# salute-developers/GigaAM

Measured on NVIDIA H100. Metric: utterances/sec (10 s audio, v2_ctc), higher is better.
Workload: dtype f16 tensor-core operands, f32 accumulate/residual/norm/head

## Files before the change

### gigaam_b200/csrc/attention_sm90.cu

```cuda
#include "kernels.h"
#include "launch.cuh"
#include "ptx.cuh"

namespace gam {
namespace {

constexpr int kMaxKB = 6;
constexpr int kTileBytes = 128 * 128;
constexpr int kThreads = 256;
constexpr float kLazyLog2 = 8.0f;
constexpr int kBarBytes = 128;

__device__ __forceinline__ float ex2(float x) {
  float y;
  asm("ex2.approx.ftz.f32 %0, %1;" : "=f"(y) : "f"(x));
  return y;
}

struct AttnParams {
  int T, nkb;
  const int* klen;
  const int* cu;
  __half* out;
  int ld_out, dk;
  float scale_log2;
};

template <int KS>
__global__ void __launch_bounds__(kThreads) attention_kernel(const __grid_constant__ CUtensorMap tmap_qkv, const AttnParams p) {
  extern __shared__ uint8_t smem_raw[];
  uint8_t* smem = reinterpret_cast<uint8_t*>((reinterpret_cast<uintptr_t>(smem_raw) + 1023) & ~uintptr_t(1023));
  const int nst = min(p.nkb, kMaxKB);
  uint8_t* sQ = smem;
  uint8_t* sK = smem + kTileBytes;
  uint8_t* sV = sK + nst * kTileBytes;
  uint64_t* bars = reinterpret_cast<uint64_t*>(sV + nst * kTileBytes);
  uint64_t* q_full = bars;
  uint64_t* kv_full = bars + 1;

  const int qt = blockIdx.x, h = blockIdx.y, b = blockIdx.z;
  const int klen = p.klen != nullptr ? min(max(__ldg(p.klen + b), 0), p.T) : p.T;
  const int kb_valid = (klen + 127) >> 7;
  if (p.cu != nullptr && qt >= kb_valid) return;
  const int row0 = p.cu != nullptr ? __ldg(p.cu + b) : b * p.T;
  const int qlim = p.cu != nullptr ? klen : p.T;
  const int nk = max(1, kb_valid);
  const int dmodel = p.ld_out;

  auto issue_block = [&](int kb, int st) {
    ptx::mbar_arrive_expect_tx(&kv_full[st], 2 * kTileBytes);
    ptx::tma_load_2d(sK + st * kTileBytes, &tmap_qkv, &kv_full[st], dmodel + h * p.dk, row0 + kb * 128);
    ptx::tma_load_2d(sV + st * kTileBytes, &tmap_qkv, &kv_full[st], 2 * dmodel + h * p.dk, row0 + kb * 128);
  };
  if (threadIdx.x == 0) {
    const int npre = nk < kMaxKB ? nk : kMaxKB;
    ptx::prefetch_tmap(&tmap_qkv);
    ptx::mbar_init(q_full, 1);
#pragma unroll
    for (int i = 0; i < kMaxKB; ++i)
      if (i < npre) ptx::mbar_init(&kv_full[i], 1);
    ptx::fence_mbar_init();
    ptx::mbar_arrive_expect_tx(q_full, kTileBytes);
    ptx::tma_load_2d(sQ, &tmap_qkv, q_full, h * p.dk, row0 + qt * 128);
#pragma unroll
    for (int kb = 0; kb < kMaxKB; ++kb)
      if (kb < npre) issue_block(kb, kb);
  }
  __syncthreads();

  const int warp = threadIdx.x >> 5, lane = threadIdx.x & 31;
  const int g = lane >> 2, t4 = lane & 3;
  uint32_t qa[KS][4];
  ptx::mbar_wait(q_full, 0);
#pragma unroll
  for (int kk = 0; kk < KS; ++kk)
    ptx::ldsm_x4(ptx::smem_u32(sQ) + ptx::sw128_off(warp * 16 + (lane & 15), kk * 16 + (lane >> 4) * 8), qa[kk][0], qa[kk][1],
                 qa[kk][2], qa[kk][3]);

  float o[2 * KS][4];
#pragma unroll
  for (int i = 0; i < 2 * KS; ++i) o[i][0] = o[i][1] = o[i][2] = o[i][3] = 0.f;
  float mc[2] = {0.f, 0.f};
  float sum[2] = {0.f, 0.f};

  for (int kb = 0; kb < nk; ++kb) {
    const int nvalid = max(min(klen - kb * 128, 128), 0);
    const int st = kb % kMaxKB;
    ptx::mbar_wait(&kv_full[st], (kb / kMaxKB) & 1);
    uint8_t* kt = sK + st * kTileBytes;
    uint8_t* vt = sV + st * kTileBytes;
    if (nvalid < 128) {
      __syncthreads();
      for (int i = threadIdx.x; i < (128 - nvalid) * 8; i += kThreads)
        reinterpret_cast<uint4*>(vt + nvalid * 128)[i] = make_uint4(0u, 0u, 0u, 0u);
      __syncthreads();
    }
    const int nch = (nvalid + 15) >> 4;

    float s[16][4];
#pragma unroll
    for (int j = 0; j < 8; ++j) {
      s[2 * j][0] = s[2 * j][1] = s[2 * j][2] = s[2 * j][3] = 0.f;
      s[2 * j + 1][0] = s[2 * j + 1][1] = s[2 * j + 1][2] = s[2 * j + 1][3] = 0.f;
      if (j < nch) {
#pragma unroll
        for (int kk = 0; kk < KS; ++kk) {
          uint32_t b0, b1, b2, b3;
          ptx::ldsm_x4(ptx::smem_u32(kt) + ptx::sw128_off(16 * j + (lane & 7) + ((lane >> 4) << 3), kk * 16 + ((lane >> 3) & 1) * 8),
                       b0, b1, b2, b3);
          ptx::mma_16816(s[2 * j], qa[kk], b0, b1);
          ptx::mma_16816(s[2 * j + 1], qa[kk], b2, b3);
        }
      }
    }

    float bm[2] = {-INFINITY, -INFINITY};
#pragma unroll
    for (int i = 0; i < 16; ++i) {
#pragma unroll
      for (int e = 0; e < 4; ++e)
        if (8 * i + 2 * t4 + (e & 1) < nvalid) bm[e >> 1] = fmaxf(bm[e >> 1], s[i][e]);
    }
#pragma unroll
    for (int r = 0; r < 2; ++r) {
      bm[r] = fmaxf(bm[r], __shfl_xor_sync(0xffffffffu, bm[r], 1));
      bm[r] = fmaxf(bm[r], __shfl_xor_sync(0xffffffffu, bm[r], 2));
      const float bml = bm[r] * p.scale_log2;
      if (kb == 0) {
        mc[r] = bm[r] == -INFINITY ? 0.f : bml;
      } else if (bml > mc[r] + kLazyLog2) {
        const float corr = ex2(mc[r] - bml);
        mc[r] = bml;
        sum[r] *= corr;
#pragma unroll
        for (int i = 0; i < 2 * KS; ++i) {
          o[i][2 * r] *= corr;
          o[i][2 * r + 1] *= corr;
        }
      }
    }

#pragma unroll
    for (int j = 0; j < 8; ++j) {
      if (j < nch) {
        uint32_t pa[4];
#pragma unroll
        for (int u = 0; u < 2; ++u) {
#pragma unroll
          for (int r = 0; r < 2; ++r) {
            const int key = 16 * j + 8 * u + 2 * t4;
            const float p0 = key < nvalid ? ex2(fmaf(s[2 * j + u][2 * r], p.scale_log2, -mc[r])) : 0.f;
            const float p1 = key + 1 < nvalid ? ex2(fmaf(s[2 * j + u][2 * r + 1], p.scale_log2, -mc[r])) : 0.f;
            const __half2 hh = __floats2half2_rn(p0, p1);
            const float2 pr = __half22float2(hh);
            sum[r] += pr.x + pr.y;
            pa[2 * u + r] = *reinterpret_cast<const uint32_t*>(&hh);
          }
        }
#pragma unroll
        for (int dd = 0; dd < KS; ++dd) {
          uint32_t b0, b1, b2, b3;
          ptx::ldsm_x4_t(ptx::smem_u32(vt) + ptx::sw128_off(16 * j + (lane & 7) + (((lane >> 3) & 1) << 3), dd * 16 + ((lane >> 4) << 3)),
                         b0, b1, b2, b3);
          ptx::mma_16816(o[2 * dd], pa, b0, b1);
          ptx::mma_16816(o[2 * dd + 1], pa, b2, b3);
        }
      }
    }
    if (kb + kMaxKB < nk) {
      __syncthreads();
      if (threadIdx.x == 0) issue_block(kb + kMaxKB, st);
    }
  }

#pragma unroll
  for (int r = 0; r < 2; ++r) {
    sum[r] += __shfl_xor_sync(0xffffffffu, sum[r], 1);
    sum[r] += __shfl_xor_sync(0xffffffffu, sum[r], 2);
    const float inv = sum[r] > 0.f ? 1.0f / sum[r] : 0.f;
    const int q = qt * 128 + warp * 16 + g + 8 * r;
    if (q < qlim) {
      __half* dst = p.out + (static_cast<size_t>(row0) + q) * p.ld_out + h * p.dk + 2 * t4;
#pragma unroll
      for (int i = 0; i < 2 * KS; ++i) {
        const __half2 hh = __floats2half2_rn(o[i][2 * r] * inv, o[i][2 * r + 1] * inv);
        *reinterpret_cast<__half2*>(dst + 8 * i) = hh;
      }
    }
  }
}

template <int KS>
int launch_ks(const CUtensorMap* tmap_qkv, const AttnParams& p, int B, int H, cudaStream_t s) {
  const int smem = (1 + 2 * (p.nkb < kMaxKB ? p.nkb : kMaxKB)) * kTileBytes + kBarBytes + 1024;
  static PerDeviceOnce attr_once;
  if (attr_once.first() &&
      cudaFuncSetAttribute(attention_kernel<KS>, cudaFuncAttributeMaxDynamicSharedMemorySize, (1 + 2 * kMaxKB) * kTileBytes + kBarBytes + 1024) !=
          cudaSuccess)
    return -2;
  return launch_k(attention_kernel<KS>, dim3(p.nkb, H, B), dim3(kThreads), smem, s, *tmap_qkv, p) == cudaSuccess ? 0 : -2;
}

}

int launch_attention(const CUtensorMap* tmap_qkv, const int* klen, const int* cu, __half* out, int B, int T, int H, int dk,
                     int d_model, cudaStream_t s) {
  const int nkb = (T + 127) / 128;
  if (nkb <= 0 || dk % 16 != 0 || dk > 48 || (cu != nullptr && klen == nullptr)) return -1;
  AttnParams p;
  p.T = T;
  p.nkb = nkb;
  p.klen = klen;
  p.cu = cu;
  p.out = out;
  p.ld_out = d_model;
  p.dk = dk;
  p.scale_log2 = 1.4426950408889634f / sqrtf(static_cast<float>(dk));
  switch (dk / 16) {
    case 1: return launch_ks<1>(tmap_qkv, p, B, H, s);
    case 2: return launch_ks<2>(tmap_qkv, p, B, H, s);
    default: return launch_ks<3>(tmap_qkv, p, B, H, s);
  }
}

}
```

### gigaam_b200/csrc/ptx.cuh

```cuda
#pragma once
#include <cuda.h>
#include <cuda_fp16.h>
#include <cuda_runtime.h>
#include <stdint.h>

namespace gam {
namespace ptx {

__device__ __forceinline__ uint32_t smem_u32(const void* p) {
  return static_cast<uint32_t>(__cvta_generic_to_shared(p));
}

__device__ __forceinline__ uint32_t lane_id() {
  uint32_t l;
  asm volatile("mov.u32 %0, %%laneid;" : "=r"(l));
  return l;
}

__device__ __forceinline__ bool elect_one() {
  uint32_t pred = 0;
  asm volatile(
      "{\n\t"
      ".reg .pred P;\n\t"
      "elect.sync _|P, 0xffffffff;\n\t"
      "selp.u32 %0, 1, 0, P;\n\t"
      "}\n"
      : "=r"(pred));
  return pred != 0;
}

__device__ __forceinline__ void mbar_init(uint64_t* bar, uint32_t count) {
  asm volatile("mbarrier.init.shared::cta.b64 [%0], %1;" ::"r"(smem_u32(bar)), "r"(count));
}
__device__ __forceinline__ void fence_mbar_init() {
  asm volatile("fence.mbarrier_init.release.cluster;" ::: "memory");
}
__device__ __forceinline__ void fence_proxy_async_smem() {
  asm volatile("fence.proxy.async.shared::cta;" ::: "memory");
}
__device__ __forceinline__ void mbar_arrive(uint64_t* bar) {
  asm volatile("mbarrier.arrive.shared::cta.b64 _, [%0];" ::"r"(smem_u32(bar)) : "memory");
}
__device__ __forceinline__ void mbar_arrive_expect_tx(uint64_t* bar, uint32_t bytes) {
  asm volatile("mbarrier.arrive.expect_tx.shared::cta.b64 _, [%0], %1;" ::"r"(smem_u32(bar)),
               "r"(bytes)
               : "memory");
}
__device__ __forceinline__ bool mbar_try_wait(uint64_t* bar, uint32_t parity) {
  uint32_t ok;
  asm volatile(
      "{\n\t"
      ".reg .pred P;\n\t"
      "mbarrier.try_wait.parity.shared::cta.b64 P, [%1], %2;\n\t"
      "selp.u32 %0, 1, 0, P;\n\t"
      "}\n"
      : "=r"(ok)
      : "r"(smem_u32(bar)), "r"(parity)
      : "memory");
  return ok != 0;
}
__device__ __forceinline__ void mbar_wait(uint64_t* bar, uint32_t parity) {
  while (!mbar_try_wait(bar, parity)) {
  }
}

__device__ __forceinline__ void prefetch_tmap(const CUtensorMap* m) {
  asm volatile("prefetch.tensormap [%0];" ::"l"(reinterpret_cast<uint64_t>(m)) : "memory");
}
__device__ __forceinline__ void tma_load_2d(void* smem, const CUtensorMap* m, uint64_t* bar, int c0,
                                            int c1) {
  asm volatile(
      "cp.async.bulk.tensor.2d.shared::cluster.global.mbarrier::complete_tx::bytes [%0], [%1, {%3, "
      "%4}], [%2];" ::"r"(smem_u32(smem)),
      "l"(reinterpret_cast<uint64_t>(m)), "r"(smem_u32(bar)), "r"(c0), "r"(c1)
      : "memory");
}
__device__ __forceinline__ void tma_load_2d_multicast(void* smem, const CUtensorMap* m, uint64_t* bar, int c0, int c1,
                                                      uint16_t cta_mask) {
  asm volatile(
      "cp.async.bulk.tensor.2d.shared::cluster.global.mbarrier::complete_tx::bytes.multicast::cluster [%0], [%1, {%3, "
      "%4}], [%2], %5;" ::"r"(smem_u32(smem)),
      "l"(reinterpret_cast<uint64_t>(m)), "r"(smem_u32(bar)), "r"(c0), "r"(c1), "h"(cta_mask)
      : "memory");
}
__device__ __forceinline__ void tma_load_3d(void* smem, const CUtensorMap* m, uint64_t* bar, int c0, int c1, int c2) {
  asm volatile(
      "cp.async.bulk.tensor.3d.shared::cluster.global.mbarrier::complete_tx::bytes [%0], [%1, {%3, "
      "%4, %5}], [%2];" ::"r"(smem_u32(smem)),
      "l"(reinterpret_cast<uint64_t>(m)), "r"(smem_u32(bar)), "r"(c0), "r"(c1), "r"(c2)
      : "memory");
}

__device__ __forceinline__ void tma_load_4d(void* smem, const CUtensorMap* m, uint64_t* bar, int c0,
                                            int c1, int c2, int c3) {
  asm volatile(
      "cp.async.bulk.tensor.4d.shared::cluster.global.mbarrier::complete_tx::bytes [%0], [%1, {%3, "
      "%4, %5, %6}], [%2];" ::"r"(smem_u32(smem)),
      "l"(reinterpret_cast<uint64_t>(m)), "r"(smem_u32(bar)), "r"(c0), "r"(c1), "r"(c2), "r"(c3)
      : "memory");
}
__device__ __forceinline__ void tma_store_2d(const CUtensorMap* m, const void* smem, int c0, int c1) {
  asm volatile(
      "cp.async.bulk.tensor.2d.global.shared::cta.bulk_group [%0, {%2, %3}], [%1];" ::"l"(
          reinterpret_cast<uint64_t>(m)),
      "r"(smem_u32(smem)), "r"(c0), "r"(c1)
      : "memory");
}
__device__ __forceinline__ void tma_store_commit() {
  asm volatile("cp.async.bulk.commit_group;" ::: "memory");
}
template <int N>
__device__ __forceinline__ void tma_store_wait_read() {
  asm volatile("cp.async.bulk.wait_group.read %0;" ::"n"(N) : "memory");
}
template <int N>
__device__ __forceinline__ void tma_store_wait() {
  asm volatile("cp.async.bulk.wait_group %0;" ::"n"(N) : "memory");
}

template <int N>
__device__ __forceinline__ void named_bar_sync(int id) {
  asm volatile("bar.sync %0, %1;" ::"r"(id), "n"(N) : "memory");
}

template <int kRegs>
__device__ __forceinline__ void setmaxnreg_dec() {
  asm volatile("setmaxnreg.dec.sync.aligned.u32 %0;" ::"n"(kRegs));
}
template <int kRegs>
__device__ __forceinline__ void setmaxnreg_inc() {
  asm volatile("setmaxnreg.inc.sync.aligned.u32 %0;" ::"n"(kRegs));
}

__device__ __forceinline__ uint32_t mapa_u32(uint32_t smem_addr, uint32_t cta) {
  uint32_t r;
  asm volatile("mapa.shared::cluster.u32 %0, %1, %2;" : "=r"(r) : "r"(smem_addr), "r"(cta));
  return r;
}
__device__ __forceinline__ uint32_t cluster_ctarank() {
  uint32_t r;
  asm volatile("mov.u32 %0, %%cluster_ctarank;" : "=r"(r));
  return r;
}
__device__ __forceinline__ void cluster_sync() {
  asm volatile("barrier.cluster.arrive.release.aligned;\n\tbarrier.cluster.wait.acquire.aligned;" ::: "memory");
}
__device__ __forceinline__ void mbar_arrive_cluster(uint64_t* bar, uint32_t cta) {
  asm volatile("mbarrier.arrive.shared::cluster.b64 _, [%0];" ::"r"(mapa_u32(smem_u32(bar), cta)) : "memory");
}
__device__ __forceinline__ void st_async_v4(uint32_t remote_addr, uint32_t remote_bar, uint32_t a, uint32_t b, uint32_t c,
                                            uint32_t d) {
  asm volatile("st.async.weak.shared::cluster.mbarrier::complete_tx::bytes.v4.b32 [%0], {%1, %2, %3, %4}, [%5];" ::"r"(remote_addr),
               "r"(a), "r"(b), "r"(c), "r"(d), "r"(remote_bar)
               : "memory");
}
__device__ __forceinline__ uint64_t make_wgmma_desc_sw128(uint32_t smem_addr) {
  uint64_t d = 0;
  d |= static_cast<uint64_t>((smem_addr & 0x3FFFF) >> 4);
  d |= static_cast<uint64_t>(1) << 16;
  d |= static_cast<uint64_t>(1024 >> 4) << 32;
  d |= static_cast<uint64_t>(1) << 62;
  return d;
}
__device__ __forceinline__ void wgmma_fence() { asm volatile("wgmma.fence.sync.aligned;" ::: "memory"); }
__device__ __forceinline__ void wgmma_commit() { asm volatile("wgmma.commit_group.sync.aligned;" ::: "memory"); }
template <int N>
__device__ __forceinline__ void wgmma_wait() {
  asm volatile("wgmma.wait_group.sync.aligned %0;" ::"n"(N) : "memory");
}
__device__ __forceinline__ void wgmma_m64n256k16_f16(float* d, uint64_t desc_a, uint64_t desc_b, uint32_t scale_d) {
  asm volatile(
      "{\n\t"
      ".reg .pred p;\n\t"
      "setp.ne.b32 p, %130, 0;\n\t"
      "wgmma.mma_async.sync.aligned.m64n256k16.f32.f16.f16 "
      "{%0, %1, %2, %3, %4, %5, %6, %7, %8, %9, %10, %11, %12, %13, %14, %15, %16, %17, %18, %19, %20, %21, %22, %23, %24, %25, %26, %27, %28, %29, %30, %31, %32, %33, %34, %35, %36, %37, %38, %39, %40, %41, %42, %43, %44, %45, %46, %47, %48, %49, %50, %51, %52, %53, %54, %55, %56, %57, %58, %59, %60, %61, %62, %63, %64, %65, %66, %67, %68, %69, %70, %71, %72, %73, %74, %75, %76, %77, %78, %79, %80, %81, %82, %83, %84, %85, %86, %87, %88, %89, %90, %91, %92, %93, %94, %95, %96, %97, %98, %99, %100, %101, %102, %103, %104, %105, %106, %107, %108, %109, %110, %111, %112, %113, %114, %115, %116, %117, %118, %119, %120, %121, %122, %123, %124, %125, %126, %127}, "
      "%128, %129, p, 1, 1, 0, 0;\n\t"
      "}\n"
      : "+f"(d[0]), "+f"(d[1]), "+f"(d[2]), "+f"(d[3]), "+f"(d[4]), "+f"(d[5]), "+f"(d[6]), "+f"(d[7]), "+f"(d[8]), "+f"(d[9]), "+f"(d[10]), "+f"(d[11]), "+f"(d[12]), "+f"(d[13]), "+f"(d[14]), "+f"(d[15]), "+f"(d[16]), "+f"(d[17]), "+f"(d[18]), "+f"(d[19]), "+f"(d[20]), "+f"(d[21]), "+f"(d[22]), "+f"(d[23]), "+f"(d[24]), "+f"(d[25]), "+f"(d[26]), "+f"(d[27]), "+f"(d[28]), "+f"(d[29]), "+f"(d[30]), "+f"(d[31]), "+f"(d[32]), "+f"(d[33]), "+f"(d[34]), "+f"(d[35]), "+f"(d[36]), "+f"(d[37]), "+f"(d[38]), "+f"(d[39]), "+f"(d[40]), "+f"(d[41]), "+f"(d[42]), "+f"(d[43]), "+f"(d[44]), "+f"(d[45]), "+f"(d[46]), "+f"(d[47]), "+f"(d[48]), "+f"(d[49]), "+f"(d[50]), "+f"(d[51]), "+f"(d[52]), "+f"(d[53]), "+f"(d[54]), "+f"(d[55]), "+f"(d[56]), "+f"(d[57]), "+f"(d[58]), "+f"(d[59]), "+f"(d[60]), "+f"(d[61]), "+f"(d[62]), "+f"(d[63]), "+f"(d[64]), "+f"(d[65]), "+f"(d[66]), "+f"(d[67]), "+f"(d[68]), "+f"(d[69]), "+f"(d[70]), "+f"(d[71]), "+f"(d[72]), "+f"(d[73]), "+f"(d[74]), "+f"(d[75]), "+f"(d[76]), "+f"(d[77]), "+f"(d[78]), "+f"(d[79]), "+f"(d[80]), "+f"(d[81]), "+f"(d[82]), "+f"(d[83]), "+f"(d[84]), "+f"(d[85]), "+f"(d[86]), "+f"(d[87]), "+f"(d[88]), "+f"(d[89]), "+f"(d[90]), "+f"(d[91]), "+f"(d[92]), "+f"(d[93]), "+f"(d[94]), "+f"(d[95]), "+f"(d[96]), "+f"(d[97]), "+f"(d[98]), "+f"(d[99]), "+f"(d[100]), "+f"(d[101]), "+f"(d[102]), "+f"(d[103]), "+f"(d[104]), "+f"(d[105]), "+f"(d[106]), "+f"(d[107]), "+f"(d[108]), "+f"(d[109]), "+f"(d[110]), "+f"(d[111]), "+f"(d[112]), "+f"(d[113]), "+f"(d[114]), "+f"(d[115]), "+f"(d[116]), "+f"(d[117]), "+f"(d[118]), "+f"(d[119]), "+f"(d[120]), "+f"(d[121]), "+f"(d[122]), "+f"(d[123]), "+f"(d[124]), "+f"(d[125]), "+f"(d[126]), "+f"(d[127])
      : "l"(desc_a), "l"(desc_b), "r"(scale_d));
}

__device__ __forceinline__ void ldsm_x4(uint32_t addr, uint32_t& r0, uint32_t& r1, uint32_t& r2, uint32_t& r3) {
  asm volatile("ldmatrix.sync.aligned.m8n8.x4.shared.b16 {%0, %1, %2, %3}, [%4];"
               : "=r"(r0), "=r"(r1), "=r"(r2), "=r"(r3)
               : "r"(addr));
}
__device__ __forceinline__ void ldsm_x4_t(uint32_t addr, uint32_t& r0, uint32_t& r1, uint32_t& r2, uint32_t& r3) {
  asm volatile("ldmatrix.sync.aligned.m8n8.x4.trans.shared.b16 {%0, %1, %2, %3}, [%4];"
               : "=r"(r0), "=r"(r1), "=r"(r2), "=r"(r3)
               : "r"(addr));
}
__device__ __forceinline__ void mma_16816(float* d, const uint32_t* a, uint32_t b0, uint32_t b1) {
  asm volatile(
      "mma.sync.aligned.m16n8k16.row.col.f32.f16.f16.f32 {%0, %1, %2, %3}, {%4, %5, %6, %7}, {%8, %9}, "
      "{%0, %1, %2, %3};"
      : "+f"(d[0]), "+f"(d[1]), "+f"(d[2]), "+f"(d[3])
      : "r"(a[0]), "r"(a[1]), "r"(a[2]), "r"(a[3]), "r"(b0), "r"(b1));
}
__device__ __forceinline__ uint32_t sw128_off(int row, int col) {
  return static_cast<uint32_t>(row * 128 + ((((col >> 3) ^ row) & 7) << 4));
}
__device__ __forceinline__ uint32_t sw128_off_f32(int row, int col) {
  return static_cast<uint32_t>(row * 128 + ((((col >> 2) ^ row) & 7) << 4));
}

}
}
```

Measured before the change: 2774.

## Rewrite attention as persistent warp-specialized WGMMA kernel with TMA producer warp

The attention kernel now runs as a persistent grid sized to SM occupancy. One producer warpgroup streams double-buffered Q tiles and a 6-stage K/V ring via TMA, synchronised with full/empty mbarriers. Two consumer warpgroups compute QK^T and PV with wgmma (PV takes the A operand from registers), and the next block's QK^T is issued before the softmax of the current one so they overlap. This removes per-CTA launch overhead, block-wide syncthreads and ldmatrix+mma.sync issue costs, at the price of register pressure (240 regs per consumer thread), one CTA per SM, and more complex phase bookkeeping.

```diff
diff --git a/gigaam_b200/csrc/attention_sm90.cu b/gigaam_b200/csrc/attention_sm90.cu
--- a/gigaam_b200/csrc/attention_sm90.cu
+++ b/gigaam_b200/csrc/attention_sm90.cu
@@ -5,11 +5,12 @@
 namespace gam {
 namespace {
 
-constexpr int kMaxKB = 6;
+constexpr int kStages = 6;
 constexpr int kTileBytes = 128 * 128;
-constexpr int kThreads = 256;
+constexpr int kThreads = 384;
 constexpr float kLazyLog2 = 8.0f;
 constexpr int kBarBytes = 128;
+constexpr int kSmemBytes = (2 + 2 * kStages) * kTileBytes + kBarBytes + 1024;
 
 __device__ __forceinline__ float ex2(float x) {
   float y;
@@ -18,7 +19,7 @@
 }
 
 struct AttnParams {
-  int T, nkb;
+  int T, nkb, H, n_items;
   const int* klen;
   const int* cu;
   __half* out;
@@ -26,179 +27,241 @@
   float scale_log2;
 };
 
+struct Item {
+  int h, qt, klen, row0, qlim, nk;
+};
+struct ItemLens {
+  int klen, cu;
+};
+__device__ __forceinline__ ItemLens item_lens(const AttnParams& p, int item) {
+  ItemLens l{p.T, 0};
+  if (item < p.n_items) {
+    const int b = item / p.nkb / p.H;
+    if (p.klen != nullptr) l.klen = __ldg(p.klen + b);
+    if (p.cu != nullptr) l.cu = __ldg(p.cu + b);
+  }
+  return l;
+}
+__device__ __forceinline__ bool item_at(const AttnParams& p, int item, const ItemLens& l, Item& it) {
+  const int bh = item / p.nkb;
+  const int b = bh / p.H;
+  it.qt = item - bh * p.nkb;
+  it.h = bh - b * p.H;
+  it.klen = min(max(l.klen, 0), p.T);
+  const int kb_valid = (it.klen + 127) >> 7;
+  if (p.cu != nullptr && it.qt >= kb_valid) return false;
+  it.row0 = p.cu != nullptr ? l.cu : b * p.T;
+  it.qlim = p.cu != nullptr ? it.klen : p.T;
+  it.nk = max(1, kb_valid);
+  return true;
+}
+
 template <int KS>
-__global__ void __launch_bounds__(kThreads) attention_kernel(const __grid_constant__ CUtensorMap tmap_qkv, const AttnParams p) {
+__global__ void __launch_bounds__(kThreads, 1) attention_kernel(const __grid_constant__ CUtensorMap tmap_qkv, const AttnParams p) {
   extern __shared__ uint8_t smem_raw[];
   uint8_t* smem = reinterpret_cast<uint8_t*>((reinterpret_cast<uintptr_t>(smem_raw) + 1023) & ~uintptr_t(1023));
-  const int nst = min(p.nkb, kMaxKB);
   uint8_t* sQ = smem;
-  uint8_t* sK = smem + kTileBytes;
-  uint8_t* sV = sK + nst * kTileBytes;
-  uint64_t* bars = reinterpret_cast<uint64_t*>(sV + nst * kTileBytes);
+  uint8_t* sK = smem + 2 * kTileBytes;
+  uint8_t* sV = sK + kStages * kTileBytes;
+  uint64_t* bars = reinterpret_cast<uint64_t*>(sV + kStages * kTileBytes);
   uint64_t* q_full = bars;
-  uint64_t* kv_full = bars + 1;
-
-  const int qt = blockIdx.x, h = blockIdx.y, b = blockIdx.z;
-  const int klen = p.klen != nullptr ? min(max(__ldg(p.klen + b), 0), p.T) : p.T;
-  const int kb_valid = (klen + 127) >> 7;
-  if (p.cu != nullptr && qt >= kb_valid) return;
-  const int row0 = p.cu != nullptr ? __ldg(p.cu + b) : b * p.T;
-  const int qlim = p.cu != nullptr ? klen : p.T;
-  const int nk = max(1, kb_valid);
-  const int dmodel = p.ld_out;
-
-  auto issue_block = [&](int kb, int st) {
-    ptx::mbar_arrive_expect_tx(&kv_full[st], 2 * kTileBytes);
-    ptx::tma_load_2d(sK + st * kTileBytes, &tmap_qkv, &kv_full[st], dmodel + h * p.dk, row0 + kb * 128);
-    ptx::tma_load_2d(sV + st * kTileBytes, &tmap_qkv, &kv_full[st], 2 * dmodel + h * p.dk, row0 + kb * 128);
-  };
-  if (threadIdx.x == 0) {
-    const int npre = nk < kMaxKB ? nk : kMaxKB;
+  uint64_t* q_empty = bars + 2;
+  uint64_t* kv_full = bars + 4;
+  uint64_t* kv_empty = kv_full + kStages;
+
+  const int warp = threadIdx.x >> 5;
+  if (warp == 0 && ptx::elect_one()) {
     ptx::prefetch_tmap(&tmap_qkv);
-    ptx::mbar_init(q_full, 1);
-#pragma unroll
-    for (int i = 0; i < kMaxKB; ++i)
-      if (i < npre) ptx::mbar_init(&kv_full[i], 1);
+    for (int i = 0; i < 2; ++i) {
+      ptx::mbar_init(&q_full[i], 1);
+      ptx::mbar_init(&q_empty[i], 2);
+    }
+    for (int s = 0; s < kStages; ++s) {
+      ptx::mbar_init(&kv_full[s], 1);
+      ptx::mbar_init(&kv_empty[s], 2);
+    }
     ptx::fence_mbar_init();
-    ptx::mbar_arrive_expect_tx(q_full, kTileBytes);
-    ptx::tma_load_2d(sQ, &tmap_qkv, q_full, h * p.dk, row0 + qt * 128);
-#pragma unroll
-    for (int kb = 0; kb < kMaxKB; ++kb)
-      if (kb < npre) issue_block(kb, kb);
   }
   __syncthreads();
 
-  const int warp = threadIdx.x >> 5, lane = threadIdx.x & 31;
+  if (warp < 4) {
+    ptx::setmaxnreg_dec<24>();
+    if (warp == 0 && ptx::elect_one()) {
+      int qs = 0, st = 0;
+      uint32_t qph = 0, kph = 0;
+      ItemLens next = item_lens(p, blockIdx.x);
+      for (int item = blockIdx.x; item < p.n_items; item += gridDim.x) {
+        const ItemLens lens = next;
+        next = item_lens(p, item + gridDim.x);
+        Item it;
+        if (!item_at(p, item, lens, it)) continue;
+        ptx::mbar_wait(&q_empty[qs], qph ^ 1);
+        ptx::mbar_arrive_expect_tx(&q_full[qs], kTileBytes);
+        ptx::tma_load_2d(sQ + qs * kTileBytes, &tmap_qkv, &q_full[qs], it.h * p.dk, it.row0 + it.qt * 128);
+        if (++qs == 2) { qs = 0; qph ^= 1; }
+        for (int kb = 0; kb < it.nk; ++kb) {
+          ptx::mbar_wait(&kv_empty[st], kph ^ 1);
+          ptx::mbar_arrive_expect_tx(&kv_full[st], 2 * kTileBytes);
+          ptx::tma_load_2d(sK + st * kTileBytes, &tmap_qkv, &kv_full[st], p.ld_out + it.h * p.dk, it.row0 + kb * 128);
+          ptx::tma_load_2d(sV + st * kTileBytes, &tmap_qkv, &kv_full[st], 2 * p.ld_out + it.h * p.dk, it.row0 + kb * 128);
+          if (++st == kStages) { st = 0; kph ^= 1; }
+        }
+      }
+    }
+    return;
+  }
+
+  ptx::setmaxnreg_inc<240>();
+  const int wg = (warp >> 2) - 1;
+  const int ctid = threadIdx.x - 128;
+  const int lane = threadIdx.x & 31;
   const int g = lane >> 2, t4 = lane & 3;
-  uint32_t qa[KS][4];
-  ptx::mbar_wait(q_full, 0);
-#pragma unroll
-  for (int kk = 0; kk < KS; ++kk)
-    ptx::ldsm_x4(ptx::smem_u32(sQ) + ptx::sw128_off(warp * 16 + (lane & 15), kk * 16 + (lane >> 4) * 8), qa[kk][0], qa[kk][1],
-                 qa[kk][2], qa[kk][3]);
-
-  float o[2 * KS][4];
-#pragma unroll
-  for (int i = 0; i < 2 * KS; ++i) o[i][0] = o[i][1] = o[i][2] = o[i][3] = 0.f;
-  float mc[2] = {0.f, 0.f};
-  float sum[2] = {0.f, 0.f};
-
-  for (int kb = 0; kb < nk; ++kb) {
-    const int nvalid = max(min(klen - kb * 128, 128), 0);
-    const int st = kb % kMaxKB;
-    ptx::mbar_wait(&kv_full[st], (kb / kMaxKB) & 1);
-    uint8_t* kt = sK + st * kTileBytes;
-    uint8_t* vt = sV + st * kTileBytes;
-    if (nvalid < 128) {
-      __syncthreads();
-      for (int i = threadIdx.x; i < (128 - nvalid) * 8; i += kThreads)
-        reinterpret_cast<uint4*>(vt + nvalid * 128)[i] = make_uint4(0u, 0u, 0u, 0u);
-      __syncthreads();
-    }
-    const int nch = (nvalid + 15) >> 4;
-
-    float s[16][4];
-#pragma unroll
-    for (int j = 0; j < 8; ++j) {
-      s[2 * j][0] = s[2 * j][1] = s[2 * j][2] = s[2 * j][3] = 0.f;
-      s[2 * j + 1][0] = s[2 * j + 1][1] = s[2 * j + 1][2] = s[2 * j + 1][3] = 0.f;
-      if (j < nch) {
-#pragma unroll
-        for (int kk = 0; kk < KS; ++kk) {
-          uint32_t b0, b1, b2, b3;
-          ptx::ldsm_x4(ptx::smem_u32(kt) + ptx::sw128_off(16 * j + (lane & 7) + ((lane >> 4) << 3), kk * 16 + ((lane >> 3) & 1) * 8),
-                       b0, b1, b2, b3);
-          ptx::mma_16816(s[2 * j], qa[kk], b0, b1);
-          ptx::mma_16816(s[2 * j + 1], qa[kk], b2, b3);
-        }
-      }
-    }
-
-    float bm[2] = {-INFINITY, -INFINITY};
-#pragma unroll
-    for (int i = 0; i < 16; ++i) {
-#pragma unroll
-      for (int e = 0; e < 4; ++e)
-        if (8 * i + 2 * t4 + (e & 1) < nvalid) bm[e >> 1] = fmaxf(bm[e >> 1], s[i][e]);
-    }
-#pragma unroll
-    for (int r = 0; r < 2; ++r) {
-      bm[r] = fmaxf(bm[r], __shfl_xor_sync(0xffffffffu, bm[r], 1));
-      bm[r] = fmaxf(bm[r], __shfl_xor_sync(0xffffffffu, bm[r], 2));
-      const float bml = bm[r] * p.scale_log2;
-      if (kb == 0) {
-        mc[r] = bm[r] == -INFINITY ? 0.f : bml;
-      } else if (bml > mc[r] + kLazyLog2) {
-        const float corr = ex2(mc[r] - bml);
-        mc[r] = bml;
-        sum[r] *= corr;
-#pragma unroll
-        for (int i = 0; i < 2 * KS; ++i) {
-          o[i][2 * r] *= corr;
-          o[i][2 * r + 1] *= corr;
-        }
-      }
-    }
-
-#pragma unroll
-    for (int j = 0; j < 8; ++j) {
-      if (j < nch) {
-        uint32_t pa[4];
+  const bool wg_leader = (threadIdx.x & 127) == 0;
+  const int lrow = wg * 64 + (warp & 3) * 16 + g;
+  int qs = 0, st = 0;
+  uint32_t qph = 0, kph = 0;
+  ItemLens next = item_lens(p, blockIdx.x);
+  for (int item = blockIdx.x; item < p.n_items; item += gridDim.x) {
+    const ItemLens lens = next;
+    next = item_lens(p, item + gridDim.x);
+    Item it;
+    if (!item_at(p, item, lens, it)) continue;
+    ptx::mbar_wait(&q_full[qs], qph);
+    const uint32_t q_addr = ptx::smem_u32(sQ + qs * kTileBytes + wg * 64 * 128);
+
+    float o[8 * KS];
+#pragma unroll
+    for (int i = 0; i < 8 * KS; ++i) o[i] = 0.f;
+    float mc[2] = {0.f, 0.f};
+    float sum[2] = {0.f, 0.f};
+
+    auto issue_s = [&](float* s, int stage) {
+      const uint32_t k_addr = ptx::smem_u32(sK + stage * kTileBytes);
+      ptx::wgmma_fence();
+#pragma unroll
+      for (int kk = 0; kk < KS; ++kk)
+        ptx::wgmma_m64n128k16_f16(s, ptx::make_wgmma_desc_sw128(q_addr + kk * 32), ptx::make_wgmma_desc_sw128(k_addr + kk * 32),
+                                  kk != 0 ? 1u : 0u);
+      ptx::wgmma_commit();
+    };
+    auto block = [&](int kb, float* s, float* s_next) {
+      int nst = st + 1;
+      uint32_t nph = kph;
+      if (nst == kStages) { nst = 0; nph ^= 1; }
+      if (kb + 1 < it.nk) {
+        ptx::mbar_wait(&kv_full[nst], nph);
+        issue_s(s_next, nst);
+      }
+      const int nvalid = max(min(it.klen - kb * 128, 128), 0);
+
+      float bm[2] = {-INFINITY, -INFINITY};
+#pragma unroll
+      for (int i = 0; i < 16; ++i) {
+#pragma unroll
+        for (int e = 0; e < 4; ++e)
+          if (8 * i + 2 * t4 + (e & 1) < nvalid) bm[e >> 1] = fmaxf(bm[e >> 1], s[4 * i + e]);
+      }
+#pragma unroll
+      for (int r = 0; r < 2; ++r) {
+        bm[r] = fmaxf(bm[r], __shfl_xor_sync(0xffffffffu, bm[r], 1));
+        bm[r] = fmaxf(bm[r], __shfl_xor_sync(0xffffffffu, bm[r], 2));
+        const float bml = bm[r] * p.scale_log2;
+        if (kb == 0) {
+          mc[r] = bm[r] == -INFINITY ? 0.f : bml;
+        } else if (bml > mc[r] + kLazyLog2) {
+          const float corr = ex2(mc[r] - bml);
+          mc[r] = bml;
+          sum[r] *= corr;
+#pragma unroll
+          for (int i = 0; i < 2 * KS; ++i) {
+            o[4 * i + 2 * r] *= corr;
+            o[4 * i + 2 * r + 1] *= corr;
+          }
+        }
+      }
+
+      uint32_t pa[32];
+#pragma unroll
+      for (int j = 0; j < 8; ++j) {
 #pragma unroll
         for (int u = 0; u < 2; ++u) {
 #pragma unroll
           for (int r = 0; r < 2; ++r) {
             const int key = 16 * j + 8 * u + 2 * t4;
-            const float p0 = key < nvalid ? ex2(fmaf(s[2 * j + u][2 * r], p.scale_log2, -mc[r])) : 0.f;
-            const float p1 = key + 1 < nvalid ? ex2(fmaf(s[2 * j + u][2 * r + 1], p.scale_log2, -mc[r])) : 0.f;
+            const float p0 = key < nvalid ? ex2(fmaf(s[4 * (2 * j + u) + 2 * r], p.scale_log2, -mc[r])) : 0.f;
+            const float p1 = key + 1 < nvalid ? ex2(fmaf(s[4 * (2 * j + u) + 2 * r + 1], p.scale_log2, -mc[r])) : 0.f;
             const __half2 hh = __floats2half2_rn(p0, p1);
             const float2 pr = __half22float2(hh);
             sum[r] += pr.x + pr.y;
-            pa[2 * u + r] = *reinterpret_cast<const uint32_t*>(&hh);
+            pa[4 * j + 2 * u + r] = *reinterpret_cast<const uint32_t*>(&hh);
           }
         }
-#pragma unroll
-        for (int dd = 0; dd < KS; ++dd) {
-          uint32_t b0, b1, b2, b3;
-          ptx::ldsm_x4_t(ptx::smem_u32(vt) + ptx::sw128_off(16 * j + (lane & 7) + (((lane >> 3) & 1) << 3), dd * 16 + ((lane >> 4) << 3)),
-                         b0, b1, b2, b3);
-          ptx::mma_16816(o[2 * dd], pa, b0, b1);
-          ptx::mma_16816(o[2 * dd + 1], pa, b2, b3);
-        }
-      }
-    }
-    if (kb + kMaxKB < nk) {
-      __syncthreads();
-      if (threadIdx.x == 0) issue_block(kb + kMaxKB, st);
-    }
-  }
-
-#pragma unroll
-  for (int r = 0; r < 2; ++r) {
-    sum[r] += __shfl_xor_sync(0xffffffffu, sum[r], 1);
-    sum[r] += __shfl_xor_sync(0xffffffffu, sum[r], 2);
-    const float inv = sum[r] > 0.f ? 1.0f / sum[r] : 0.f;
-    const int q = qt * 128 + warp * 16 + g + 8 * r;
-    if (q < qlim) {
-      __half* dst = p.out + (static_cast<size_t>(row0) + q) * p.ld_out + h * p.dk + 2 * t4;
-#pragma unroll
-      for (int i = 0; i < 2 * KS; ++i) {
-        const __half2 hh = __floats2half2_rn(o[i][2 * r] * inv, o[i][2 * r + 1] * inv);
-        *reinterpret_cast<__half2*>(dst + 8 * i) = hh;
+      }
+
+      uint8_t* vt = sV + st * kTileBytes;
+      if (nvalid < 128) {
+        for (int i = ctid; i < (128 - nvalid) * 8; i += 256) reinterpret_cast<uint4*>(vt + nvalid * 128)[i] = make_uint4(0u, 0u, 0u, 0u);
+        ptx::fence_proxy_async_smem();
+        ptx::named_bar_sync<256>(1);
+      }
+
+      const uint32_t v_addr = ptx::smem_u32(vt);
+      ptx::wgmma_fence();
+#pragma unroll
+      for (int j = 0; j < 8; ++j) ptx::wgmma_m64nNk16_f16_rs_tb<16 * KS>(o, pa + 4 * j, ptx::make_wgmma_desc_sw128(v_addr + j * 16 * 128));
+      ptx::wgmma_commit();
+      ptx::wgmma_wait<0>();
+#pragma unroll
+      for (int i = 0; i < 8 * KS; ++i) asm volatile("" : "+f"(o[i])::"memory");
+#pragma unroll
+      for (int i = 0; i < 64; ++i) asm volatile("" : "+f"(s_next[i])::"memory");
+      if (wg_leader) ptx::mbar_arrive(&kv_empty[st]);
+      st = nst;
+      kph = nph;
+    };
+
+    float sa[64], sb[64];
+    ptx::mbar_wait(&kv_full[st], kph);
+    issue_s(sa, st);
+    ptx::wgmma_wait<0>();
+#pragma unroll
+    for (int i = 0; i < 64; ++i) asm volatile("" : "+f"(sa[i])::"memory");
+    for (int kb = 0; kb < it.nk; kb += 2) {
+      block(kb, sa, sb);
+      if (kb + 1 < it.nk) block(kb + 1, sb, sa);
+    }
+    if (wg_leader) ptx::mbar_arrive(&q_empty[qs]);
+    if (++qs == 2) { qs = 0; qph ^= 1; }
+
+#pragma unroll
+    for (int r = 0; r < 2; ++r) {
+      sum[r] += __shfl_xor_sync(0xffffffffu, sum[r], 1);
+      sum[r] += __shfl_xor_sync(0xffffffffu, sum[r], 2);
+      const float inv = sum[r] > 0.f ? 1.0f / sum[r] : 0.f;
+      const int q = it.qt * 128 + lrow + 8 * r;
+      if (q < it.qlim) {
+        __half* dst = p.out + (static_cast<size_t>(it.row0) + q) * p.ld_out + it.h * p.dk + 2 * t4;
+#pragma unroll
+        for (int i = 0; i < 2 * KS; ++i) {
+          const __half2 hh = __floats2half2_rn(o[4 * i + 2 * r] * inv, o[4 * i + 2 * r + 1] * inv);
+          *reinterpret_cast<__half2*>(dst + 8 * i) = hh;
+        }
       }
     }
   }
 }
 
 template <int KS>
-int launch_ks(const CUtensorMap* tmap_qkv, const AttnParams& p, int B, int H, cudaStream_t s) {
-  const int smem = (1 + 2 * (p.nkb < kMaxKB ? p.nkb : kMaxKB)) * kTileBytes + kBarBytes + 1024;
+int launch_ks(const CUtensorMap* tmap_qkv, const AttnParams& p, cudaStream_t s) {
+  auto kern = attention_kernel<KS>;
   static PerDeviceOnce attr_once;
-  if (attr_once.first() &&
-      cudaFuncSetAttribute(attention_kernel<KS>, cudaFuncAttributeMaxDynamicSharedMemorySize, (1 + 2 * kMaxKB) * kTileBytes + kBarBytes + 1024) !=
-          cudaSuccess)
+  if (attr_once.first() && cudaFuncSetAttribute(kern, cudaFuncAttributeMaxDynamicSharedMemorySize, kSmemBytes) != cudaSuccess) return -2;
+  int dev = 0, sms = 0, per_sm = 0;
+  if (cudaGetDevice(&dev) != cudaSuccess || cudaDeviceGetAttribute(&sms, cudaDevAttrMultiProcessorCount, dev) != cudaSuccess ||
+      cudaOccupancyMaxActiveBlocksPerMultiprocessor(&per_sm, kern, kThreads, kSmemBytes) != cudaSuccess || per_sm <= 0)
     return -2;
-  return launch_k(attention_kernel<KS>, dim3(p.nkb, H, B), dim3(kThreads), smem, s, *tmap_qkv, p) == cudaSuccess ? 0 : -2;
+  const int grid = p.n_items < sms * per_sm ? p.n_items : sms * per_sm;
+  return launch_k(kern, dim3(grid), dim3(kThreads), kSmemBytes, s, *tmap_qkv, p) == cudaSuccess ? 0 : -2;
 }
 
 }
@@ -210,6 +273,8 @@
   AttnParams p;
   p.T = T;
   p.nkb = nkb;
+  p.H = H;
+  p.n_items = B * H * nkb;
   p.klen = klen;
   p.cu = cu;
   p.out = out;
@@ -217,10 +282,10 @@
   p.dk = dk;
   p.scale_log2 = 1.4426950408889634f / sqrtf(static_cast<float>(dk));
   switch (dk / 16) {
-    case 1: return launch_ks<1>(tmap_qkv, p, B, H, s);
-    case 2: return launch_ks<2>(tmap_qkv, p, B, H, s);
-    default: return launch_ks<3>(tmap_qkv, p, B, H, s);
-  }
-}
-
-}
+    case 1: return launch_ks<1>(tmap_qkv, p, s);
+    case 2: return launch_ks<2>(tmap_qkv, p, s);
+    default: return launch_ks<3>(tmap_qkv, p, s);
+  }
+}
+
+}
diff --git a/gigaam_b200/csrc/ptx.cuh b/gigaam_b200/csrc/ptx.cuh
--- a/gigaam_b200/csrc/ptx.cuh
+++ b/gigaam_b200/csrc/ptx.cuh
@@ -180,6 +180,42 @@
       : "+f"(d[0]), "+f"(d[1]), "+f"(d[2]), "+f"(d[3]), "+f"(d[4]), "+f"(d[5]), "+f"(d[6]), "+f"(d[7]), "+f"(d[8]), "+f"(d[9]), "+f"(d[10]), "+f"(d[11]), "+f"(d[12]), "+f"(d[13]), "+f"(d[14]), "+f"(d[15]), "+f"(d[16]), "+f"(d[17]), "+f"(d[18]), "+f"(d[19]), "+f"(d[20]), "+f"(d[21]), "+f"(d[22]), "+f"(d[23]), "+f"(d[24]), "+f"(d[25]), "+f"(d[26]), "+f"(d[27]), "+f"(d[28]), "+f"(d[29]), "+f"(d[30]), "+f"(d[31]), "+f"(d[32]), "+f"(d[33]), "+f"(d[34]), "+f"(d[35]), "+f"(d[36]), "+f"(d[37]), "+f"(d[38]), "+f"(d[39]), "+f"(d[40]), "+f"(d[41]), "+f"(d[42]), "+f"(d[43]), "+f"(d[44]), "+f"(d[45]), "+f"(d[46]), "+f"(d[47]), "+f"(d[48]), "+f"(d[49]), "+f"(d[50]), "+f"(d[51]), "+f"(d[52]), "+f"(d[53]), "+f"(d[54]), "+f"(d[55]), "+f"(d[56]), "+f"(d[57]), "+f"(d[58]), "+f"(d[59]), "+f"(d[60]), "+f"(d[61]), "+f"(d[62]), "+f"(d[63]), "+f"(d[64]), "+f"(d[65]), "+f"(d[66]), "+f"(d[67]), "+f"(d[68]), "+f"(d[69]), "+f"(d[70]), "+f"(d[71]), "+f"(d[72]), "+f"(d[73]), "+f"(d[74]), "+f"(d[75]), "+f"(d[76]), "+f"(d[77]), "+f"(d[78]), "+f"(d[79]), "+f"(d[80]), "+f"(d[81]), "+f"(d[82]), "+f"(d[83]), "+f"(d[84]), "+f"(d[85]), "+f"(d[86]), "+f"(d[87]), "+f"(d[88]), "+f"(d[89]), "+f"(d[90]), "+f"(d[91]), "+f"(d[92]), "+f"(d[93]), "+f"(d[94]), "+f"(d[95]), "+f"(d[96]), "+f"(d[97]), "+f"(d[98]), "+f"(d[99]), "+f"(d[100]), "+f"(d[101]), "+f"(d[102]), "+f"(d[103]), "+f"(d[104]), "+f"(d[105]), "+f"(d[106]), "+f"(d[107]), "+f"(d[108]), "+f"(d[109]), "+f"(d[110]), "+f"(d[111]), "+f"(d[112]), "+f"(d[113]), "+f"(d[114]), "+f"(d[115]), "+f"(d[116]), "+f"(d[117]), "+f"(d[118]), "+f"(d[119]), "+f"(d[120]), "+f"(d[121]), "+f"(d[122]), "+f"(d[123]), "+f"(d[124]), "+f"(d[125]), "+f"(d[126]), "+f"(d[127])
       : "l"(desc_a), "l"(desc_b), "r"(scale_d));
 }
+__device__ __forceinline__ void wgmma_m64n128k16_f16(float* d, uint64_t desc_a, uint64_t desc_b, uint32_t scale_d) {
+  asm volatile(
+      "{\n\t"
+      ".reg .pred p;\n\t"
+      "setp.ne.b32 p, %66, 0;\n\t"
+      "wgmma.mma_async.sync.aligned.m64n128k16.f32.f16.f16 "
+      "{%0, %1, %2, %3, %4, %5, %6, %7, %8, %9, %10, %11, %12, %13, %14, %15, %16, %17, %18, %19, %20, %21, %22, %23, %24, %25, %26, %27, %28, %29, %30, %31, %32, %33, %34, %35, %36, %37, %38, %39, %40, %41, %42, %43, %44, %45, %46, %47, %48, %49, %50, %51, %52, %53, %54, %55, %56, %57, %58, %59, %60, %61, %62, %63}, "
+      "%64, %65, p, 1, 1, 0, 0;\n\t"
+      "}\n"
+      : "+f"(d[0]), "+f"(d[1]), "+f"(d[2]), "+f"(d[3]), "+f"(d[4]), "+f"(d[5]), "+f"(d[6]), "+f"(d[7]), "+f"(d[8]), "+f"(d[9]), "+f"(d[10]), "+f"(d[11]), "+f"(d[12]), "+f"(d[13]), "+f"(d[14]), "+f"(d[15]), "+f"(d[16]), "+f"(d[17]), "+f"(d[18]), "+f"(d[19]), "+f"(d[20]), "+f"(d[21]), "+f"(d[22]), "+f"(d[23]), "+f"(d[24]), "+f"(d[25]), "+f"(d[26]), "+f"(d[27]), "+f"(d[28]), "+f"(d[29]), "+f"(d[30]), "+f"(d[31]), "+f"(d[32]), "+f"(d[33]), "+f"(d[34]), "+f"(d[35]), "+f"(d[36]), "+f"(d[37]), "+f"(d[38]), "+f"(d[39]), "+f"(d[40]), "+f"(d[41]), "+f"(d[42]), "+f"(d[43]), "+f"(d[44]), "+f"(d[45]), "+f"(d[46]), "+f"(d[47]), "+f"(d[48]), "+f"(d[49]), "+f"(d[50]), "+f"(d[51]), "+f"(d[52]), "+f"(d[53]), "+f"(d[54]), "+f"(d[55]), "+f"(d[56]), "+f"(d[57]), "+f"(d[58]), "+f"(d[59]), "+f"(d[60]), "+f"(d[61]), "+f"(d[62]), "+f"(d[63])
+      : "l"(desc_a), "l"(desc_b), "r"(scale_d));
+}
+template <int N>
+__device__ __forceinline__ void wgmma_m64nNk16_f16_rs_tb(float* d, const uint32_t* a, uint64_t desc_b) {
+  static_assert(N == 16 || N == 32 || N == 48, "m64nNk16 wrapper: N must be 16, 32 or 48");
+  if constexpr (N == 16) {
+    asm volatile(
+        "wgmma.mma_async.sync.aligned.m64n16k16.f32.f16.f16 "
+        "{%0, %1, %2, %3, %4, %5, %6, %7}, {%8, %9, %10, %11}, %12, 1, 1, 1, 1;\n"
+        : "+f"(d[0]), "+f"(d[1]), "+f"(d[2]), "+f"(d[3]), "+f"(d[4]), "+f"(d[5]), "+f"(d[6]), "+f"(d[7])
+        : "r"(a[0]), "r"(a[1]), "r"(a[2]), "r"(a[3]), "l"(desc_b));
+  } else if constexpr (N == 32) {
+    asm volatile(
+        "wgmma.mma_async.sync.aligned.m64n32k16.f32.f16.f16 "
+        "{%0, %1, %2, %3, %4, %5, %6, %7, %8, %9, %10, %11, %12, %13, %14, %15}, {%16, %17, %18, %19}, %20, 1, 1, 1, 1;\n"
+        : "+f"(d[0]), "+f"(d[1]), "+f"(d[2]), "+f"(d[3]), "+f"(d[4]), "+f"(d[5]), "+f"(d[6]), "+f"(d[7]), "+f"(d[8]), "+f"(d[9]), "+f"(d[10]), "+f"(d[11]), "+f"(d[12]), "+f"(d[13]), "+f"(d[14]), "+f"(d[15])
+        : "r"(a[0]), "r"(a[1]), "r"(a[2]), "r"(a[3]), "l"(desc_b));
+  } else {
+    asm volatile(
+        "wgmma.mma_async.sync.aligned.m64n48k16.f32.f16.f16 "
+        "{%0, %1, %2, %3, %4, %5, %6, %7, %8, %9, %10, %11, %12, %13, %14, %15, %16, %17, %18, %19, %20, %21, %22, %23}, "
+        "{%24, %25, %26, %27}, %28, 1, 1, 1, 1;\n"
+        : "+f"(d[0]), "+f"(d[1]), "+f"(d[2]), "+f"(d[3]), "+f"(d[4]), "+f"(d[5]), "+f"(d[6]), "+f"(d[7]), "+f"(d[8]), "+f"(d[9]), "+f"(d[10]), "+f"(d[11]), "+f"(d[12]), "+f"(d[13]), "+f"(d[14]), "+f"(d[15]), "+f"(d[16]), "+f"(d[17]), "+f"(d[18]), "+f"(d[19]), "+f"(d[20]), "+f"(d[21]), "+f"(d[22]), "+f"(d[23])
+        : "r"(a[0]), "r"(a[1]), "r"(a[2]), "r"(a[3]), "l"(desc_b));
+  }
+}
 
 __device__ __forceinline__ void ldsm_x4(uint32_t addr, uint32_t& r0, uint32_t& r1, uint32_t& r2, uint32_t& r3) {
   asm volatile("ldmatrix.sync.aligned.m8n8.x4.shared.b16 {%0, %1, %2, %3}, [%4];"
```

Result: no change. 2771, median of 6 (-0.1%).
